# Improbable-AI/walk-these-ways

Hardware: AMD Instinct MI355X
Metric: env-steps/sec (sim+PPO) (higher is better)
Workload: dtype f32

## Files before the change

walk-these-ways_amd/csrc/go1ppo.hip:

```cpp
#include <hip/hip_runtime.h>
#include <stdint.h>
#include <string.h>
#include "../../include/go1ppo.h"

typedef uint16_t bf16_t;
static_assert(sizeof(Go1PpoAdamExtras) == 56 && sizeof(Go1PpoGemmArgs) == 96 && sizeof(Go1PpoWgradProblem) == 96 && sizeof(Go1PpoGradPiece) == 56, "ctypes mirrors (fused.py) assume these sizes");
typedef __attribute__((ext_vector_type(4))) float f32x4;

__device__ __forceinline__ float bf2f(bf16_t u) { return __uint_as_float(((uint32_t)u) << 16); }
__device__ __forceinline__ bf16_t f2bf(float f) {
  return __builtin_bit_cast(bf16_t, (__bf16)f);
}
struct alignas(16) Bf8 { bf16_t v[8]; };

typedef __attribute__((ext_vector_type(4))) uint32_t u32x4_t;
__device__ __forceinline__ void put16_wt(void* p, u32x4_t v) {
  asm volatile("global_store_dwordx4 %0, %1, off sc1\n\ts_nop 1" : : "v"((__attribute__((address_space(1))) void*)p), "v"(v) : "memory");
}
__device__ __forceinline__ void put16_wt(void* p, const Bf8& v) { put16_wt(p, __builtin_bit_cast(u32x4_t, v)); }
__device__ __forceinline__ void put16_wt(void* p, f32x4 v) { put16_wt(p, __builtin_bit_cast(u32x4_t, v)); }
__device__ __forceinline__ void put16_wt(void* p, uint4 v) { put16_wt(p, u32x4_t{v.x, v.y, v.z, v.w}); }

__device__ __forceinline__ float elu1(float x) {
  float em = x > -1e-3f ? fmaf(0.5f * x, x, x) : __expf(x) - 1.f;
// ... 501 lines not shown
  wgrad2_body((const bf16_t*)P.dz, P.ld_dz, (const bf16_t*)P.h, P.ld_h, m_begin, m_end, P.dW, P.ldw, P.bias_grad, n0, k0,
              P.bias_grad && k0 == 0, T, P.zero_n, P.zero_k0, P.zero_k1);
}

__global__ __launch_bounds__(256) void act_kernel(const bf16_t* mean, const bf16_t* value, int head_ld, const float* std, int A,
                                                  int64_t rows, const float* noise, float* actions, float* mu, float* sigma,
                                                  float* values, float* logp) {
  int64_t r = (int64_t)blockIdx.x * blockDim.x + threadIdx.x;
  if (r >= rows) return;
  const float HALF_LOG_2PI = 0.9189385332046727f;
  float lp = 0.f, logs = 0.f;
  for (int j = 0; j < A; j++) {
    float sg = std[j], m = bf2f(mean[r * head_ld + j]);
    float a = m + sg * noise[r * A + j];
    float z = (a - m) / sg;
    lp += -0.5f * z * z;
    logs += logf(sg);
    actions[r * A + j] = a;
    mu[r * A + j] = m;
    sigma[r * A + j] = sg;
  }
  logp[r] = lp - (logs + A * HALF_LOG_2PI);
  values[r] = bf2f(value[r * head_ld]);
}

__global__ __launch_bounds__(256) void store_step_kernel(const float* rewards, const uint8_t* dones, const uint8_t* time_outs,
                                                         const int32_t* env_bins, const float* values, float gamma, int64_t n,
                                                         float* rewards_out, uint8_t* dones_out, float* env_bins_out) {
  int64_t i = (int64_t)blockIdx.x * 256 + threadIdx.x;
  if (i >= n) return;
  float r = rewards[i];
  if (time_outs) r += gamma * (values[i] * (time_outs[i] ? 1.f : 0.f));
  rewards_out[i] = r;
  dones_out[i] = dones[i];
  if (env_bins) env_bins_out[i] = (float)env_bins[i];
}

__global__ __launch_bounds__(256) void gae_kernel(const float* rewards, const uint8_t* dones, const float* values, const float* last_values,
                                                  int T, int64_t N, float gamma, float lam, float* returns, float* advantages, double* stats) {
  __shared__ double red[2][4];
  int64_t e = (int64_t)blockIdx.x * 256 + threadIdx.x;
  double s1 = 0.0, s2 = 0.0;
  if (e < N) {
    float adv = 0.f, next_v = last_values[e];
    for (int t = T - 1; t >= 0; t--) {
      const int64_t i = (int64_t)t * N + e;
      const float alive = 1.f - (float)dones[i];
      const float v = values[i];
      const float delta = rewards[i] + alive * gamma * next_v - v;
      adv = delta + alive * gamma * lam * adv;
      const float ret = adv + v;
      const float a = ret - v;
      returns[i] = ret;
      advantages[i] = a;
      s1 += a;
      s2 += (double)a * a;
      next_v = v;
    }
  }
  for (int o = 32; o > 0; o >>= 1) { s1 += __shfl_xor(s1, o, 64); s2 += __shfl_xor(s2, o, 64); }
  if ((threadIdx.x & 63) == 0) { red[0][threadIdx.x >> 6] = s1; red[1][threadIdx.x >> 6] = s2; }
  __syncthreads();
  if (threadIdx.x < 2) det_put(det_gae_slab + (int64_t)blockIdx.x * 2 + threadIdx.x, red[threadIdx.x][0] + red[threadIdx.x][1] + red[threadIdx.x][2] + red[threadIdx.x][3]);
  if (!det_last(&det_count[DET_GAE], gridDim.x)) return;
  if (threadIdx.x < 2) {
    double t = 0.0;
#pragma unroll 16
    for (unsigned b = 0; b < gridDim.x; b++) t += det_gae_slab[(int64_t)b * 2 + threadIdx.x];
    stats[threadIdx.x] += t;
  }
}

__global__ __launch_bounds__(256) void normalize_kernel(float* adv, int64_t n, const double* stats) {
  int64_t i = (int64_t)blockIdx.x * 256 + threadIdx.x;
  if (i >= n) return;
  const double cnt = stats[2], mean = stats[0] / cnt;
  double var = (stats[1] - cnt * mean * mean) / (cnt - 1.0);
  var = var > 0.0 ? var : 0.0;
  const float m = (float)mean, sd = (float)sqrt(var);
  adv[i] = (adv[i] - m) / (sd + 1e-8f);
}

#define OPT_BLOCKS 2048
template <bool NORM>
__device__ __forceinline__ float grad_pieces_pass(float* g, int64_t n, const Go1PpoGradPiece* __restrict__ pieces, int num_pieces, float gscale) {
  const int64_t tid = (int64_t)blockIdx.x * 256 + threadIdx.x, nth = (int64_t)gridDim.x * 256;
  auto gap_groups = [&](int64_t lo, int64_t hi) -> int64_t { return NORM && hi > lo ? (hi - lo + 7) >> 3 : 0; };
  auto piece_groups = [&](const Go1PpoGradPiece& P) -> int64_t { return P.kind == 0 ? gap_groups(P.begin, P.begin + P.count) : P.count >> 3; };
  int64_t total = 0;
  {
    int64_t cur = 0;
    for (int q = 0; q <= num_pieces; q++) {
      const int64_t pb = q < num_pieces ? pieces[q].begin : n;
      total += gap_groups(cur, pb < n ? pb : n);
      if (q == num_pieces) break;
      total += piece_groups(pieces[q]);
      cur = pieces[q].begin + pieces[q].count;
    }
  }
  float s = 0.f;
  auto plain8 = [&](int64_t i, int64_t hi) {
    if (i + 8 <= hi) {
      const f32x4 a = reinterpret_cast<const f32x4*>(g + i)[0] * gscale, b = reinterpret_cast<const f32x4*>(g + i)[1] * gscale;
#pragma unroll
      for (int e = 0; e < 4; e++) { s = fmaf(a[e], a[e], s); s = fmaf(b[e], b[e], s); }
    } else {
      for (int64_t j = i; j < hi; j++) { const float x = g[j] * gscale; s = fmaf(x, x, s); }
    }
  };
  for (int64_t f = tid; f < total; f += nth) {
    int64_t cum = 0, cur = 0;
    for (int q = 0; q <= num_pieces; q++) {
      const int64_t pb = q < num_pieces ? pieces[q].begin : n, ge = pb < n ? pb : n;
      const int64_t gg = gap_groups(cur, ge);
      if (f >= cum && f < cum + gg) plain8(cur + ((f - cum) << 3), ge);
      cum += gg;
      if (q == num_pieces) break;
      const Go1PpoGradPiece P = pieces[q];
      const int64_t pg = piece_groups(P);
      cur = P.begin + P.count;
      if (f >= cum && f < cum + pg) {
        const int64_t i = (f - cum) << 3;
        if (P.kind == 0) plain8(P.begin + i, cur);
        else {
          float acc[8] = {0.f, 0.f, 0.f, 0.f, 0.f, 0.f, 0.f, 0.f};
          if (P.kind == 1) {
            const float* src = (const float*)P.src + i;
            int b = 0;
            for (; b + 4 <= P.slabs; b += 4) {
              f32x4 lo[4], hi[4];
#pragma unroll
              for (int u = 0; u < 4; u++) {
                lo[u] = reinterpret_cast<const f32x4*>(src + (int64_t)(b + u) * P.stride)[0];
                hi[u] = reinterpret_cast<const f32x4*>(src + (int64_t)(b + u) * P.stride)[1];
              }
#pragma unroll
              for (int u = 0; u < 4; u++)
#pragma unroll
                for (int e = 0; e < 4; e++) { acc[e] += lo[u][e]; acc[4 + e] += hi[u][e]; }
            }
            for (; b < P.slabs; b++) {
              const f32x4 lo = reinterpret_cast<const f32x4*>(src + (int64_t)b * P.stride)[0], hi = reinterpret_cast<const f32x4*>(src + (int64_t)b * P.stride)[1];
#pragma unroll
              for (int e = 0; e < 4; e++) { acc[e] += lo[e]; acc[4 + e] += hi[e]; }
            }
          } else {
            const bf16_t* src = (const bf16_t*)P.src + i;
            int b = 0;
            for (; b + 4 <= P.slabs; b += 4) {
              Bf8 v[4];
#pragma unroll
              for (int u = 0; u < 4; u++) v[u] = *reinterpret_cast<const Bf8*>(src + (int64_t)(b + u) * P.stride);
#pragma unroll
              for (int u = 0; u < 4; u++)
#pragma unroll
                for (int e = 0; e < 8; e++) acc[e] += bf2f(v[u].v[e]);
            }
            for (; b < P.slabs; b++) {
              const Bf8 v = *reinterpret_cast<const Bf8*>(src + (int64_t)b * P.stride);
#pragma unroll
              for (int e = 0; e < 8; e++) acc[e] += bf2f(v.v[e]);
            }
          }
          if (P.zero_rows > 0) {
            const int64_t row = i / P.cols;
            const int c = (int)(i - row * P.cols);
            if (row < P.zero_rows && c < P.zero_c1 && c + 8 > P.zero_c0) {
#pragma unroll
              for (int e = 0; e < 8; e++)
                if (c + e >= P.zero_c0 && c + e < P.zero_c1) acc[e] = 0.f;
            }
          }
          float* out = g + P.begin + i;
          reinterpret_cast<f32x4*>(out)[0] = f32x4{acc[0], acc[1], acc[2], acc[3]};
          reinterpret_cast<f32x4*>(out)[1] = f32x4{acc[4], acc[5], acc[6], acc[7]};
          if (NORM) {
#pragma unroll
            for (int e = 0; e < 8; e++) { const float x = acc[e] * gscale; s = fmaf(x, x, s); }
          }
        }
      }
      cum += pg;
    }
  }
  return s;
}
__global__ __launch_bounds__(256) void grad_reduce_kernel(float* g, const Go1PpoGradPiece* __restrict__ pieces, int num_pieces) {
  grad_pieces_pass<false>(g, 0, pieces, num_pieces, 1.f);
}

__global__ __launch_bounds__(256) void prestep_kernel(const float* g, int64_t n, float gscale, float* partial, float* step, float* lr,
                                                      const float* kl, float kl_scale, float desired_kl, float lr_min, float lr_max,
                                                      const Go1PpoGradPiece* __restrict__ pieces, int num_pieces) {
  __shared__ float red[4];
  float s = 0.f;
  if (partial && pieces) {
    s = grad_pieces_pass<true>(const_cast<float*>(g), n, pieces, num_pieces, gscale);
    for (int o = 32; o > 0; o >>= 1) s += __shfl_xor(s, o, 64);
    if ((threadIdx.x & 63) == 0) red[threadIdx.x >> 6] = s;
    __syncthreads();
    if (threadIdx.x == 0) partial[blockIdx.x] = red[0] + red[1] + red[2] + red[3];
  } else if (partial) {
    const int64_t n4 = ((reinterpret_cast<uintptr_t>(g) & 15) == 0) ? n >> 2 : 0;
    for (int64_t i = (int64_t)blockIdx.x * 256 + threadIdx.x; i < n4; i += (int64_t)OPT_BLOCKS * 256) {
      const f32x4 x = reinterpret_cast<const f32x4*>(g)[i] * gscale;
      s = fmaf(x[0], x[0], s); s = fmaf(x[1], x[1], s); s = fmaf(x[2], x[2], s); s = fmaf(x[3], x[3], s);
    }
    for (int64_t i = 4 * n4 + (int64_t)blockIdx.x * 256 + threadIdx.x; i < n; i += (int64_t)OPT_BLOCKS * 256) {
      float x = g[i] * gscale;
      s = fmaf(x, x, s);
    }
    for (int o = 32; o > 0; o >>= 1) s += __shfl_xor(s, o, 64);
    if ((threadIdx.x & 63) == 0) red[threadIdx.x >> 6] = s;
    __syncthreads();
    if (threadIdx.x == 0) partial[blockIdx.x] = red[0] + red[1] + red[2] + red[3];
  }
  if (blockIdx.x == 0 && threadIdx.x == 0) {
    step[0] += 1.f;
    if (kl) {
      const float k = kl[0] * kl_scale, l = lr[0];
      if (k > desired_kl * 2.f) lr[0] = fmaxf(lr_min, l / 1.5f);
      else if (k < desired_kl / 2.f && k > 0.f) lr[0] = fminf(lr_max, l * 1.5f);
    }
  }
}

template <int V>
__global__ __launch_bounds__(256) void adam_kernel(float* p, float* g, float* m, float* v, int64_t start0, int64_t count0,
                                                   int64_t start1, int64_t count1, float gscale, const float* partial, float max_norm,
                                                   const float* step, const float* lr, float beta1, float beta2, float eps,
                                                   bf16_t* body, int64_t n_body, float* tail, int64_t n_tail, int zero_grad, float* zero_slot,
                                                   Go1PpoAdamExtras ex) {
  __shared__ float clip_red[4];
  float clip = 1.f;
  if (partial) {
    float s = 0.f;
#pragma unroll
    for (int u = 0; u < OPT_BLOCKS / 256; u++) s += partial[threadIdx.x + 256 * u];
    for (int o = 32; o > 0; o >>= 1) s += __shfl_xor(s, o, 64);
    if ((threadIdx.x & 63) == 0) clip_red[threadIdx.x >> 6] = s;
    __syncthreads();
    clip = fminf(1.f, max_norm / (sqrtf((clip_red[0] + clip_red[1]) + (clip_red[2] + clip_red[3])) + 1e-6f));
  }
  const float gs = gscale * clip;
  const float t = step[0], l = lr[0];
  const float bc1 = 1.f - powf(beta1, t), bc2 = 1.f - powf(beta2, t);
  const float step_size = l / bc1, inv_sqrt_bc2 = rsqrtf(bc2);
  const int64_t total = count0 + count1;
// ... 559 lines not shown
```

walk-these-ways_amd/go1_gym_learn/ppo_cse/fused.py:

```python
import ctypes
import os

import torch

HEAD = 64
_HERE = os.path.dirname(os.path.abspath(__file__))
_LIB_PATH = os.path.normpath(os.path.join(_HERE, "..", "..", "csrc", "libgo1ppo.so"))
_lib = None


class Go1PpoLibraryMissing(RuntimeError):
    pass


class LossArgs(ctypes.Structure):
    _fields_ = [("mean", ctypes.c_void_p), ("value", ctypes.c_void_p), ("std", ctypes.c_void_p),
                ("head_ld", ctypes.c_int32), ("num_actions", ctypes.c_int32), ("rows", ctypes.c_int64),
                ("idx", ctypes.c_void_p), ("actions", ctypes.c_void_p), ("old_mu", ctypes.c_void_p),
                ("old_sigma", ctypes.c_void_p), ("old_logp", ctypes.c_void_p), ("advantages", ctypes.c_void_p),
                ("returns", ctypes.c_void_p), ("old_values", ctypes.c_void_p),
                ("clip_param", ctypes.c_float), ("value_loss_coef", ctypes.c_float), ("entropy_coef", ctypes.c_float),
                ("use_clipped_value_loss", ctypes.c_int32),
                ("d_mean", ctypes.c_void_p), ("d_value", ctypes.c_void_p), ("d_std", ctypes.c_void_p),
                ("d_mean_bias", ctypes.c_void_p), ("d_value_bias", ctypes.c_void_p), ("kl", ctypes.c_void_p),
# ... 111 lines not shown
    L.go1ppo_normalize.argtypes = [vp, i64, vp, vp]
    L.go1ppo_opt_partials.argtypes = []
    L.go1ppo_opt_prestep.argtypes = [vp, i64, f32, vp, vp, vp, vp, f32, f32, f32, f32, vp]
    L.go1ppo_opt_prestep_pieces.argtypes = [vp, i64, vp, i32, f32, vp, vp, vp, vp, f32, f32, f32, f32, vp]
    L.go1ppo_grad_reduce.argtypes = [vp, vp, i32, vp]
    L.go1ppo_opt_adam.argtypes = [vp, vp, vp, vp, i64, i64, i64, i64, f32, vp, f32, vp, vp, f32, f32, f32, vp, i64, vp, i64, i32, vp,
                                  ctypes.POINTER(AdamExtras), vp]
    for name in EXPORTED_SYMBOLS[:-1]:
        getattr(L, name).restype = ctypes.c_int
    L.go1ppo_version.restype = ctypes.c_char_p
    if path is None:
        _lib = L
    return L


def _stream():
    return torch.cuda.current_stream().cuda_stream


def _chk(rc, what):
    if rc != 0:
        raise RuntimeError(f"{what} failed with code {rc}")


def _ptr(t):
    return None if t is None else t.data_ptr()


def _ld(t):
    assert t.dim() == 2 and t.stride(1) == 1
    return t.stride(0)


def gemm_args(a, b, c, bias=None, elu=None, elu_bwd_of=None, elu_skip=None):
    g = GemmArgs()
    g.A, g.B, g.C, g.bias, g.H = a.data_ptr(), b.data_ptr(), c.data_ptr(), _ptr(bias), _ptr(elu_bwd_of)
    g.M, g.N, g.K, g.lda, g.ldb, g.ldc = a.shape[0], b.shape[0], a.shape[1], _ld(a), _ld(b), _ld(c)
    assert b.shape[1] == g.K and tuple(c.shape) == (g.M, g.N) and (elu is None or elu_bwd_of is None)
    assert a.dtype == b.dtype == c.dtype == torch.bfloat16 and (bias is None or bias.dtype in (torch.float32, torch.bfloat16))
    g.bias_bf16 = int(bias is not None and bias.dtype == torch.bfloat16)
    if elu_bwd_of is not None:
        assert elu_bwd_of.shape == c.shape and elu_bwd_of.dtype == torch.bfloat16
        g.epilogue, g.ldh = 2, _ld(elu_bwd_of)
    elif elu is not None:
        g.epilogue = 1
        g.elu_c0, g.elu_c1 = (0, g.N) if elu is True else elu
        if elu_skip is not None:
            g.elu_skip_c0, g.elu_skip_c1 = elu_skip
    return g


def gemm_nt(lib, a, b, c, bias=None, elu=None, elu_bwd_of=None):
    g = gemm_args(a, b, c, bias, elu, elu_bwd_of)
    _chk(lib.go1ppo_gemm_nt(ctypes.byref(g), _stream()), "go1ppo_gemm_nt")
    return c


def gemm_nt_pair(lib, first, second):
    ga, gb = gemm_args(**first), gemm_args(**second)
    _chk(lib.go1ppo_gemm_nt_pair(ctypes.byref(ga), ctypes.byref(gb), _stream()), "go1ppo_gemm_nt_pair")


class FusedNet:

    def __init__(self, policy, body, grad, M, lib, with_grad, two_streams=True, fused_tails=None):
        assert body.dtype == torch.bfloat16 and body.is_cuda
        self.pol, self.M, self.lib = policy, M, lib
        dev = body.device
        self.P = {name: policy._block(body, name) for name, _ in policy.blocks}
        self.G = {name: policy._block(grad, name) for name, _ in policy.blocks} if grad is not None else None
        self.nd, self.na, self.nc = policy.first
        self.n1 = self.nd + self.na + self.nc
        self.depth = {n: len(l) for n, l in policy.nets.items()}
        bf = dict(device=dev, dtype=torch.bfloat16)
        self.Y1 = torch.zeros(M, self.n1, **bf)
        self.Y1d = torch.zeros(M, self.nd, **bf)
        self.Z = {n: {li: torch.zeros(M, self.P[f"{n}.{li}.W"].shape[0], **bf) for li in range(1, d)}
                  for n, d in self.depth.items()}
        assert policy.npv <= HEAD and self.P["Wz"].shape == (self.na, HEAD)
        self._recording, self._batched, self._plans = None, False, {}
        self._grad = grad
        self.defer_grad_sum = False
        self._rec_pieces, self._slab_ws, self._last_pieces = None, {}, {}
        self._wgrad_tn = M % 64 == 0
        self._tails = self._tails_ad = None
        if fused_tails is None:
            fused_tails = M <= int(os.environ.get("GO1_FUSED_TAILS_MAX_ROWS", "2048"))
        self._elu_on_load = not with_grad
        if fused_tails and self._fused_tails_ok():
            nd, na = self.nd, self.na
            eol = self._elu_on_load
            self._tails = (self._tail_args([("adaptation", self.Y1[:, :nd])], with_grad, elu_in=eol),
                           self._tail_args([("actor", self.Y1[:, nd:nd + na]), ("critic", self.Y1[:, nd + na:])], with_grad, elu_in=eol,
                                           latent_for="actor" if eol else None))
            self._tails_ad = self._tail_args([("adaptation", self.Y1d)], with_grad)
        self._mlp2 = (self._tails is None and os.environ.get("GO1_MLP2", "1") == "1" and self.nd == MLP2_DIMS[0] and
                      all(self.depth[n] >= 3 and tuple(self.P[f"{n}.{self.depth[n] - 2}.W"].shape) == (MLP2_DIMS[1], MLP2_DIMS[0])
                          and tuple(self.P[f"{n}.{self.depth[n] - 1}.W"].shape) == (MLP2_DIMS[2], MLP2_DIMS[1]) for n in self.depth)
                      and self.depth["adaptation"] == 3 and self.depth["actor"] == 4 and self.depth["critic"] == 4)
        self._mlp2_cache = {}
        self._tail_in_loss = False
        na1, nc1 = int(self.P["actor.1.W"].shape[0]), int(self.P["critic.1.W"].shape[0])
        nt_ok = all(v % 64 == 0 for v in (na1, nc1, self.na, self.n1 - self.nd - self.na)) and \
            all(self.P[k].data_ptr() % 16 == 0 for k in ("actor.1.b", "critic.1.b", "actor.1.W", "critic.1.W"))
        pair_ok = nt_ok and na1 == nc1 and self.na == self.n1 - self.nd - self.na
        self._l1_nt = nt_ok
        self._pair = pair_ok
        self._side = torch.cuda.Stream(device=dev) if two_streams else None
        if with_grad:
            self.X = torch.zeros(M, policy.Kp, **bf)
            self.dH1 = {"adaptation": torch.zeros(M, self.nd, **bf), "actor": torch.zeros(M, self.na, **bf),
                        "critic": torch.zeros(M, self.nc, **bf)}
            self.dY1 = torch.zeros(M, self.n1, **bf)
            self.dZ = {n: {li: torch.zeros_like(z) for li, z in zs.items()} for n, zs in self.Z.items()}
            w1_split = next((b for b in (M // 6144, 4, 2) if b >= 2 and M % b == 0 and (M // b) % 64 == 0), 1)
            self._w1_tmp = torch.zeros(w1_split, self.n1, policy.Kp, **bf)
            self._dgrad_nt = self._mlp2 and nt_ok
            self._WT = {n: torch.zeros(self.P[f"{n}.1.W"].shape[1], self.P[f"{n}.1.W"].shape[0], **bf) for n in ("actor", "critic")} \
                if self._dgrad_nt else None
            self._wt_by_optimizer = False
            self.priv_mask = (self.nd + self.na, policy.K + 1, policy.K + 1 + policy.npv)

    def _elu(self, y, lat=None, lat_cols=0):
        wz = self.P["Wz"] if lat is not None else None
        _chk(self.lib.go1ppo_elu_fwd(y.data_ptr(), y.shape[0], y.shape[1], _ld(y), _ptr(lat), _ld(lat) if lat is not None else 0,
                                     self.pol.npv if lat is not None else 0, _ptr(wz), HEAD, lat_cols, _stream()), "go1ppo_elu_fwd")

    def _elu_bwd(self, d, h, bias_grad, out=None):
        out = d if out is None else out
        _chk(self.lib.go1ppo_elu_bwd(d.data_ptr(), _ld(d), _ptr(h), _ld(h) if h is not None else 0, d.shape[0], d.shape[1],
                                     _ptr(bias_grad), out.data_ptr(), _ld(out), _stream()), "go1ppo_elu_bwd")

    def _wgrad(self, dz, h, gW, gb=None, zero=None):
        n, k = dz.shape[1], h.shape[1]
        assert gW.shape == (n, k) and gW.is_contiguous()
        if self._recording is not None:
            self._recording.append((dz, h, gW, gb, zero))
            return
        if self._batched:
            return
        assert zero is None or zero[0] == 0, "the structural zeros are applied by the batched launch"
        _chk(self.lib.go1ppo_wgrad(dz.data_ptr(), _ld(dz), h.data_ptr(), _ld(h), dz.shape[0], n, k, gW.data_ptr(), k, _ptr(gb),
                                   _stream()), "go1ppo_wgrad")

    def _tail_args(self, nets_and_inputs, keep_intermediates, elu_in=False, latent_for=None):
        a = TailArgs()
        a.num_nets = len(nets_and_inputs)
        for N, (net, h) in zip(a.net, nets_and_inputs):
            d = self.depth[net]
            N.in_, N.rows, N.ld_in, N.num_layers = h.data_ptr(), h.shape[0], _ld(h), d - 1
            N.elu_in = int(bool(elu_in))
            if elu_in and latent_for == net:
                lat, wz = self.Z["adaptation"][self.depth["adaptation"] - 1], self.P["Wz"]
                N.latent, N.wz, N.lat_ld, N.wz_ld, N.npv = lat.data_ptr(), wz.data_ptr(), _ld(lat), HEAD, self.pol.npv
            for li in range(1, d):
                L, W, z = N.layer[li - 1], self.P[f"{net}.{li}.W"], self.Z[net][li]
                last = li == d - 1
                L.W, L.bias = W.data_ptr(), self.P[f"{net}.{li}.b"].data_ptr()
                L.out = z.data_ptr() if (last or keep_intermediates) else None
                L.n_out, L.k_in, L.ld_out, L.elu = W.shape[0], W.shape[1], _ld(z), 0 if last else 1
        return a

    def _fused_tails_ok(self):
        ok = all(self.depth[n] - 1 <= 4 for n in self.depth)
        for n, d in self.depth.items():
            for li in range(1, d):
# ... 164 lines not shown
        nd, d, G, Z, dZ = self.nd, self.dH1["adaptation"], self.G, self.Z, self.dZ
        if not self._tail_in_loss:
            self._mlp2_bwd("adaptation_only", [("adaptation", self.Y1d, d)])
        self._wgrad(dZ["adaptation"][2], Z["adaptation"][1], G["adaptation.2.W"], None)
        self._wgrad(dZ["adaptation"][1], self.Y1d, G["adaptation.1.W"], G["adaptation.1.b"])
        self._big_wgrad(d, x, G["W1"][:nd], self._w1_tmp[:, :nd], own_kernel=self._wgrad_tn)

    def adam_transposes(self):
        if not getattr(self, "_dgrad_nt", False):
            return []
        out = []
        for n in ("actor", "critic"):
            i = self.pol.index[f"{n}.1.W"]
            rows, cols = self.pol.blocks[i][1]
            out.append((self.pol.offsets[i], rows, cols, self._WT[n]))
        return out

    def refresh_transposes(self):
        if getattr(self, "_dgrad_nt", False):
            for n in ("actor", "critic"):
                self._WT[n].copy_(self.P[f"{n}.1.W"].t())

    def _branch(self):
        if self._side is None:
            import contextlib
            return contextlib.nullcontext()
        self._side.wait_stream(torch.cuda.current_stream())
        self._forked = True
        return torch.cuda.stream(self._side)

    def _join(self):
        if self._side is not None and getattr(self, "_forked", False):
            torch.cuda.current_stream().wait_stream(self._side)
            self._forked = False

    def forward_adaptation(self, x):
        if self._mlp2:
            return self._forward_adaptation_mlp2(x)
        torch.mm(x, self.P["W1"][:self.nd].t(), out=self.Y1d)
        self._elu(self.Y1d)
        if self._tails_ad is not None:
            _chk(self.lib.go1ppo_tail_fwd(ctypes.byref(self._tails_ad), _stream()), "go1ppo_tail_fwd")
            return self.Z["adaptation"][self.depth["adaptation"] - 1]
        return self._tail("adaptation", self.Y1d)

    def _tail_bwd(self, net, h0, dh0, head_bias_done=True):
        P, G, d = self.P, self.G, self.depth[net]
        for li in range(d - 1, 0, -1):
            dz = self.dZ[net][li]
            h_in = self.Z[net][li - 1] if li > 1 else h0
            gb = None if (li == d - 1 and head_bias_done) else G[f"{net}.{li}.b"]
            self._wgrad(dz, h_in, G[f"{net}.{li}.W"], gb)
            out = self.dZ[net][li - 1] if li > 1 else dh0
            torch.mm(dz, P[f"{net}.{li}.W"], out=out)
            if li > 1:
                self._elu_bwd(out, h_in, None)

    def _big_wgrad(self, dY, x, gW, tmp, own_kernel=False):
        zr, zc0, zc1 = self.priv_mask
        zr = min(zr, gW.shape[0])
        if own_kernel:
            self._wgrad(dY, x, gW, zero=(zr, zc0, zc1))
            return
        b = tmp.shape[0]
        if b == 1 or not tmp.is_contiguous():
            torch.mm(dY.t(), x, out=tmp[0])
            part, count, stride = tmp[0], 1, gW.numel()
        else:
            torch.bmm(dY.view(b, dY.shape[0] // b, dY.shape[1]).transpose(1, 2), x.view(b, x.shape[0] // b, x.shape[1]), out=tmp)
            part, count, stride = tmp, b, tmp.stride(0)
        assert gW.is_contiguous() and part.stride(-1) == 1 and part.stride(-2) == gW.shape[1]
        if self._rec_pieces is not None:
            self._rec_pieces.append(dict(begin=self._grad_offset(gW), count=gW.numel(), src=part, stride=stride, kind=2, slabs=count,
                                         cols=gW.shape[1], zero=(zr, zc0, zc1)))

    def _grad_offset(self, view):
        off = (view.data_ptr() - self._grad.data_ptr()) // 4
        assert view.dtype == torch.float32 and view.is_contiguous() and 0 <= off and off + view.numel() <= self._grad.numel()
        return int(off)

    def last_pieces(self, kind):
        return self._last_pieces.get(kind)

    def _run_planned(self, key, fn):
        if key not in self._plans:
            self._recording, self._rec_pieces = [], []
            fn()
            rec, self._recording = self._recording, None
            pieces, self._rec_pieces = self._rec_pieces, None
            tab = (WgradProblem * len(rec))()
            for P, (dz, h, gW, gb, zero) in zip(tab, rec):
                P.dz, P.h, P.dW, P.bias_grad = dz.data_ptr(), h.data_ptr(), gW.data_ptr(), _ptr(gb)
                if zero is not None:
                    P.zero_n, P.zero_k0, P.zero_k1 = zero
                P.rows, P.ld_dz, P.ld_h, P.n, P.k, P.ldw = dz.shape[0], _ld(dz), _ld(h), dz.shape[1], h.shape[1], gW.shape[1]
            tn = self._wgrad_tn and all(P.rows % 64 == 0 and P.n % 8 == 0 and P.k % 8 == 0 for P in tab)
            plan = self.lib.go1ppo_wgrad_tn_plan if tn else self.lib.go1ppo_wgrad_plan
            if tn:
                for P, (dz, h, gW, gb, zero) in zip(tab, rec):
                    P.partials, P.partial_stride = 16, gW.numel()
            total = plan(tab, len(rec))
            if total <= 0:
                raise RuntimeError(f"go1ppo_wgrad_plan failed with code {total}")
            if tn:
                for j, (P, (dz, h, gW, gb, zero)) in enumerate(zip(tab, rec)):
                    S = -(-P.rows // P.chunk_rows)
                    ws = self._slab_ws.get((key[0], j))
                    if ws is None or tuple(ws.shape) != (S, gW.numel()):
                        ws = self._slab_ws[(key[0], j)] = torch.zeros(S, gW.numel(), device=gW.device, dtype=torch.float32)
                    P.partials, P.partial_stride = ws.data_ptr(), gW.numel()
                    pieces.append(dict(begin=self._grad_offset(gW), count=gW.numel(), src=ws, stride=gW.numel(), kind=1, slabs=S, cols=gW.shape[1],
                                       zero=(0, 0, 0)))
                if plan(tab, len(rec)) != total:
                    raise RuntimeError("go1ppo_wgrad_tn_plan: the plan changed with the slab buffers attached")
            dev = torch.frombuffer(bytearray(bytes(tab)), dtype=torch.uint8).to(self.Y1.device)
            ptab = None
            if pieces:
                pieces.sort(key=lambda q: q["begin"])
                arr = (GradPiece * len(pieces))()
                end = 0
                for A, q in zip(arr, pieces):
                    assert q["begin"] >= end and q["begin"] % 8 == 0 and q["count"] % 8 == 0 and q["stride"] % 8 == 0, "slab pieces: ascending, disjoint, multiples of 8"
                    end = q["begin"] + q["count"]
                    A.begin, A.count, A.src, A.stride, A.kind, A.slabs, A.cols = q["begin"], q["count"], q["src"].data_ptr(), q["stride"], q["kind"], q["slabs"], q["cols"]
                    A.zero_rows, A.zero_c0, A.zero_c1 = q["zero"]
                ptab = (torch.frombuffer(bytearray(bytes(arr)), dtype=torch.uint8).to(self.Y1.device), len(pieces), [q["src"] for q in pieces])
            self._plans[key] = (dev, len(rec), total, rec, tn, ptab)
        else:
            self._batched = True
            try:
                fn()
            finally:
                self._batched = False
        dev, count, total, _, tn, ptab = self._plans[key]
        launch = self.lib.go1ppo_wgrad_tn_batched if tn else self.lib.go1ppo_wgrad_batched
        _chk(launch(dev.data_ptr(), count, total, _stream()), "go1ppo_wgrad_batched")
        self._last_pieces[key[0]] = None
        if ptab is None:
            return
        if self.defer_grad_sum:
            self._last_pieces[key[0]] = ptab[:2]
        else:
            _chk(self.lib.go1ppo_grad_reduce(self._grad.data_ptr(), ptab[0].data_ptr(), ptab[1], _stream()), "go1ppo_grad_reduce")

    def backward(self, x):
        self._run_planned(("ppo", x.data_ptr()), lambda: (self._backward_mlp2 if self._mlp2 else self._backward)(x))

    def backward_adaptation(self, x):
        self._run_planned(("adaptation", x.data_ptr()), lambda: (self._backward_adaptation_mlp2 if self._mlp2 else self._backward_adaptation)(x))

    def _backward(self, x):
        nd, na = self.nd, self.na
        G, Y1, dY1, dH1 = self.G, self.Y1, self.dY1, self.dH1
        cols = {"adaptation": slice(0, nd), "actor": slice(nd, nd + na), "critic": slice(nd + na, self.n1)}
        with self._branch():
            self._tail_bwd("critic", Y1[:, cols["critic"]], dH1["critic"])
            self._elu_bwd(dH1["critic"], Y1[:, cols["critic"]], None, out=dY1[:, cols["critic"]])
        self._tail_bwd("actor", Y1[:, cols["actor"]], dH1["actor"])
        self._elu_bwd(dH1["actor"], Y1[:, cols["actor"]], None, out=dY1[:, cols["actor"]])
        last = self.depth["adaptation"] - 1
        latent, dlat = self.Z["adaptation"][last], self.dZ["adaptation"][last]
        dA1 = dY1[:, cols["actor"]]
        self._wgrad(dA1, latent, G["Wz"])
        torch.mm(dA1, self.P["Wz"], out=dlat)
        self._tail_bwd("adaptation", Y1[:, :nd], dH1["adaptation"], head_bias_done=False)
        self._elu_bwd(dH1["adaptation"], Y1[:, :nd], None, out=dY1[:, :nd])
        self._join()
        self._big_wgrad(dY1, x, G["W1"], self._w1_tmp)

    def _backward_adaptation(self, x):
        nd, d = self.nd, self.dH1["adaptation"]
        self._tail_bwd("adaptation", self.Y1d, d)
        self._elu_bwd(d, self.Y1d, None)
        self._big_wgrad(d, x, self.G["W1"][:nd], self._w1_tmp[:, :nd], own_kernel=self._wgrad_tn)

    def ppo_loss(self, st, idx, std, g_std, A, kl, acc):
        la, lc = self.depth["actor"] - 1, self.depth["critic"] - 1
        flat = lambda t: t.flatten(0, 1)
        a = LossArgs()
        a.mean, a.value, a.std = self.Z["actor"][la].data_ptr(), self.Z["critic"][lc].data_ptr(), std.data_ptr()
        a.head_ld, a.num_actions, a.rows = HEAD, std.numel(), self.M
        a.idx = idx.data_ptr()
        for field, t in (("actions", st.actions), ("old_mu", st.mu), ("old_sigma", st.sigma), ("old_logp", st.actions_log_prob),
                         ("advantages", st.advantages), ("returns", st.returns), ("old_values", st.values)):
            t = flat(t)
            assert t.is_contiguous() and t.dtype == torch.float32
            setattr(a, field, t.data_ptr())
        a.clip_param, a.value_loss_coef, a.entropy_coef = A.clip_param, A.value_loss_coef, A.entropy_coef
        a.use_clipped_value_loss = int(A.use_clipped_value_loss)
        a.d_mean, a.d_value = self.dZ["actor"][la].data_ptr(), self.dZ["critic"][lc].data_ptr()
        a.d_std = g_std.data_ptr()
        a.d_mean_bias = self.G[f"actor.{la}.b"].data_ptr()
        a.d_value_bias = self.G[f"critic.{lc}.b"].data_ptr()
        a.kl = kl.data_ptr()
        a.value_loss = acc[0:].data_ptr()
        a.surrogate_loss = acc[1:].data_ptr()
        if self._tail_in_loss:
            Z, dZ = self.Z, self.dZ
            arr = self._mlp2_tail("ac", [("actor", Z["actor"][1], dZ["actor"][1]), ("critic", Z["critic"][1], dZ["critic"][1])])
            _chk(self.lib.go1ppo_mlp2_tail_ppo(arr, ctypes.byref(a), _stream()), "go1ppo_mlp2_tail_ppo")
            return
        _chk(self.lib.go1ppo_loss(ctypes.byref(a), _stream()), "go1ppo_loss")

    def adaptation_loss(self, st, idx, num_train, selective, acc):
        last = self.depth["adaptation"] - 1
        pred, dpred = self.Z["adaptation"][last], self.dZ["adaptation"][last]
        target = st.privileged_observations.flatten(0, 1)
        assert target.is_contiguous() and target.dtype == torch.float32 and target.shape[1] == self.pol.npv
        if self._tail_in_loss:
            arr = self._mlp2_tail("adaptation_only", [("adaptation", self.Y1d, self.dH1["adaptation"])])
            q = MseArgs()
            q.target, q.idx, q.num_train, q.npv, q.selective = target.data_ptr(), idx.data_ptr(), num_train, self.pol.npv, int(selective)
            q.d_pred_bias, q.train_loss, q.test_loss = self.G[f"adaptation.{last}.b"].data_ptr(), acc[2:].data_ptr(), acc[3:].data_ptr()
            _chk(self.lib.go1ppo_mlp2_tail_mse(arr, ctypes.byref(q), _stream()), "go1ppo_mlp2_tail_mse")
            return
        _chk(self.lib.go1ppo_mse(pred.data_ptr(), HEAD, target.data_ptr(), self.pol.npv, idx.data_ptr(), self.M, num_train,
                                 int(selective), dpred.data_ptr(), self.G[f"adaptation.{last}.b"].data_ptr(),
                                 acc[2:].data_ptr(), acc[3:].data_ptr(), _stream()), "go1ppo_mse")


def act(lib, mean, value, std, noise, st, s):
    _chk(lib.go1ppo_act(mean.data_ptr(), value.data_ptr(), _ld(mean), std.data_ptr(), std.numel(), mean.shape[0], noise.data_ptr(),
                        st.actions[s].data_ptr(), st.mu[s].data_ptr(), st.sigma[s].data_ptr(), st.values[s].data_ptr(),
                        st.actions_log_prob[s].data_ptr(), _stream()), "go1ppo_act")


def store_step(lib, st, s, rewards, dones, time_outs, env_bins, gamma):
    n = rewards.shape[0]
    for t, dt in ((rewards, torch.float32), (dones, torch.uint8)):
        assert t.is_contiguous() and t.dtype == dt and t.shape[0] == n
    if time_outs is not None:
        assert time_outs.is_contiguous() and time_outs.element_size() == 1
    if env_bins is not None:
        assert env_bins.is_contiguous() and env_bins.dtype == torch.int32
    _chk(lib.go1ppo_store_step(rewards.data_ptr(), dones.data_ptr(), _ptr(time_outs), _ptr(env_bins), st.values[s].data_ptr(), gamma, n,
                               st.rewards[s].data_ptr(), st.dones[s].data_ptr(), st.env_bins[s].data_ptr() if env_bins is not None else None,
                               _stream()), "go1ppo_store_step")


def ring_step(lib, st, s, obs, privileged_obs, obs_history, X):
    N, no, H = st.num_envs, st.obs_ring.shape[2], st.history_length
    npv = st.privileged_observations.shape[-1]
    for t in (obs, privileged_obs):
        assert t.dtype == torch.float32 and t.is_contiguous() and t.shape[0] == N
    assert X.dtype == torch.bfloat16 and X.is_contiguous() and tuple(X.shape) == (N, st.padded_width)
    if s == 0:
        assert obs_history.dtype == torch.float32 and obs_history.stride(1) == 1 and tuple(obs_history.shape) == (N, H * no)
        _chk(lib.go1ppo_ring_snapshot(obs_history.data_ptr(), obs_history.stride(0), N, H, no, st.obs_ring.data_ptr(), _stream()),
             "go1ppo_ring_snapshot")
    dst = None if s == 0 else st.obs_ring[s + H - 1].data_ptr()
    _chk(lib.go1ppo_ring_step(obs.data_ptr(), privileged_obs.data_ptr(), dst, st.obs_ring[s].data_ptr(), N, H, no, npv, st.padded_width,
                              X.data_ptr(), st.observations[s].data_ptr(), st.privileged_observations[s].data_ptr(), _stream()),
         "go1ppo_ring_step")


def ring_gather(lib, st, idx, X):
    N, no, H = st.num_envs, st.obs_ring.shape[2], st.history_length
    priv = st.privileged_observations
    assert idx.dtype == torch.int64 and idx.is_contiguous() and X.is_contiguous() and tuple(X.shape) == (idx.numel(), st.padded_width)
    assert priv.dtype == torch.float32 and priv.is_contiguous()
    _chk(lib.go1ppo_ring_gather(st.obs_ring.data_ptr(), priv.data_ptr(), idx.data_ptr(), idx.numel(), N, H, no, priv.shape[-1],
                                st.padded_width, X.data_ptr(), _stream()), "go1ppo_ring_gather")


def gae(lib, st, last_values, gamma, lam, stats):
    T, N = st.num_transitions_per_env, st.num_envs
    stats.zero_()
    _chk(lib.go1ppo_gae(st.rewards.data_ptr(), st.dones.data_ptr(), st.values.data_ptr(), last_values.data_ptr(), T, N, gamma, lam,
                        st.returns.data_ptr(), st.advantages.data_ptr(), stats.data_ptr(), _stream()), "go1ppo_gae")
    stats[2] = float(T * N)


def normalize(lib, st, stats):
    _chk(lib.go1ppo_normalize(st.advantages.data_ptr(), st.advantages.numel(), stats.data_ptr(), _stream()), "go1ppo_normalize")


class FusedAdam:

    def __init__(self, lib, master, body, std, n_body, lr, ranges=None, betas=(0.9, 0.999), eps=1e-8):
        self.lib, self.master, self.body, self.std, self.n_body = lib, master, body, std, n_body
        dev = master.device
        self.m, self.v = torch.zeros_like(master), torch.zeros_like(master)
        self.step = torch.zeros(1, device=dev)
        self.lr = torch.full((1,), float(lr), device=dev)
        self.partial = torch.zeros(lib.go1ppo_opt_partials(), device=dev)
        self.betas, self.eps = betas, eps
        r = list(ranges or [(0, master.numel())]) + [(0, 0)]
        self.r0, self.r1 = r[0], r[1]
        self.n_norm = max(a + b for a, b in r)
        self.extras = AdamExtras()
        self._keep = []
# ... 35 lines not shown
```

Baseline: 5.308 million.

## Use wave-level prefix table for grad pieces and trim adaptation wgrad rows

The gradient-piece pass now builds a per-wave prefix-sum table of segment group counts using shuffles and ballots. Each wave then visits only the segments its 64 lanes cover, instead of every thread walking all pieces linearly. The zero-row division uses 32-bit math when sizes allow. Separately, the adaptation backward's weight-gradient plan limits rows to the training subset, rounded up to 64, so held-out rows are skipped; this adds plan-cache keys per row count and assumes held-out rows contribute zero gradient.

```diff
diff --git a/walk-these-ways_amd/csrc/go1ppo.hip b/walk-these-ways_amd/csrc/go1ppo.hip
--- a/walk-these-ways_amd/csrc/go1ppo.hip
+++ b/walk-these-ways_amd/csrc/go1ppo.hip
@@ -607,22 +607,44 @@
 }
 
 #define OPT_BLOCKS 2048
+__device__ __forceinline__ int64_t wave_uniform(int64_t x) {
+  return (int64_t)(((uint64_t)(uint32_t)__builtin_amdgcn_readfirstlane((int)((uint64_t)x >> 32)) << 32) |
+                   (uint32_t)__builtin_amdgcn_readfirstlane((int)(uint32_t)x));
+}
 template <bool NORM>
 __device__ __forceinline__ float grad_pieces_pass(float* g, int64_t n, const Go1PpoGradPiece* __restrict__ pieces, int num_pieces, float gscale) {
-  const int64_t tid = (int64_t)blockIdx.x * 256 + threadIdx.x, nth = (int64_t)gridDim.x * 256;
+  const int lane = threadIdx.x & 63;
+  const int64_t wave0 = (int64_t)blockIdx.x * 256 + 64 * __builtin_amdgcn_readfirstlane((int)(threadIdx.x >> 6)), nth = (int64_t)gridDim.x * 256;
   auto gap_groups = [&](int64_t lo, int64_t hi) -> int64_t { return NORM && hi > lo ? (hi - lo + 7) >> 3 : 0; };
   auto piece_groups = [&](const Go1PpoGradPiece& P) -> int64_t { return P.kind == 0 ? gap_groups(P.begin, P.begin + P.count) : P.count >> 3; };
-  int64_t total = 0;
-  {
-    int64_t cur = 0;
+  auto gap_lo = [&](int q) -> int64_t { return q ? pieces[q - 1].begin + pieces[q - 1].count : 0; };
+  auto gap_hi = [&](int q) -> int64_t { const int64_t pb = q < num_pieces ? pieces[q].begin : n; return pb < n ? pb : n; };
+  const bool table = num_pieces < 64;
+  int64_t total = 0, gstart = 0, pstart = 0;
+  if (table) {
+    int64_t gg = 0, pg = 0;
+    if (lane <= num_pieces) {
+      gg = gap_groups(gap_lo(lane), gap_hi(lane));
+      if (lane < num_pieces) pg = piece_groups(pieces[lane]);
+    }
+    int64_t incl = gg + pg;
+#pragma unroll
+    for (int o = 1; o < 64; o <<= 1) {
+      const int64_t up = __shfl_up(incl, o, 64);
+      if (lane >= o) incl += up;
+    }
+    gstart = incl - (gg + pg);
+    pstart = gstart + gg;
+    total = wave_uniform(__shfl(incl, 63, 64));
+  } else {
     for (int q = 0; q <= num_pieces; q++) {
-      const int64_t pb = q < num_pieces ? pieces[q].begin : n;
-      total += gap_groups(cur, pb < n ? pb : n);
-      if (q == num_pieces) break;
-      total += piece_groups(pieces[q]);
-      cur = pieces[q].begin + pieces[q].count;
-    }
-  }
+      total += gap_groups(gap_lo(q), gap_hi(q));
+      if (q < num_pieces) total += piece_groups(pieces[q]);
+    }
+  }
+  auto segment_of = [&](int64_t f) -> int {
+    return __popcll(__ballot(gstart <= f)) + __popcll(__ballot(pstart <= f)) - 1;
+  };
   float s = 0.f;
   auto plain8 = [&](int64_t i, int64_t hi) {
     if (i + 8 <= hi) {
@@ -633,17 +655,26 @@
       for (int64_t j = i; j < hi; j++) { const float x = g[j] * gscale; s = fmaf(x, x, s); }
     }
   };
-  for (int64_t f = tid; f < total; f += nth) {
-    int64_t cum = 0, cur = 0;
-    for (int q = 0; q <= num_pieces; q++) {
-      const int64_t pb = q < num_pieces ? pieces[q].begin : n, ge = pb < n ? pb : n;
-      const int64_t gg = gap_groups(cur, ge);
-      if (f >= cum && f < cum + gg) plain8(cur + ((f - cum) << 3), ge);
-      cum += gg;
-      if (q == num_pieces) break;
+  for (int64_t f0 = wave0; f0 < total; f0 += nth) {
+    const int64_t f = f0 + lane;
+    int k0 = 0, k1 = 2 * num_pieces;
+    int64_t cum = 0;
+    if (table) {
+      k0 = segment_of(f0);
+      k1 = segment_of(f0 + 63 < total ? f0 + 63 : total - 1);
+      cum = wave_uniform(__shfl((k0 & 1) ? pstart : gstart, k0 >> 1, 64));
+    }
+    for (int k = k0; k <= k1; k++) {
+      const int q = k >> 1;
+      if (!(k & 1)) {
+        const int64_t lo = gap_lo(q), ge = gap_hi(q), gg = gap_groups(lo, ge);
+        if (f >= cum && f < cum + gg) plain8(lo + ((f - cum) << 3), ge);
+        cum += gg;
+        continue;
+      }
       const Go1PpoGradPiece P = pieces[q];
       const int64_t pg = piece_groups(P);
-      cur = P.begin + P.count;
+      const int64_t cur = P.begin + P.count;
       if (f >= cum && f < cum + pg) {
         const int64_t i = (f - cum) << 3;
         if (P.kind == 0) plain8(P.begin + i, cur);
@@ -688,7 +719,7 @@
             }
           }
           if (P.zero_rows > 0) {
-            const int64_t row = i / P.cols;
+            const int64_t row = (uint64_t)P.count >> 31 ? i / P.cols : (int64_t)((uint32_t)i / (uint32_t)P.cols);
             const int c = (int)(i - row * P.cols);
             if (row < P.zero_rows && c < P.zero_c1 && c + 8 > P.zero_c0) {
 #pragma unroll
diff --git a/walk-these-ways_amd/go1_gym_learn/ppo_cse/fused.py b/walk-these-ways_amd/go1_gym_learn/ppo_cse/fused.py
--- a/walk-these-ways_amd/go1_gym_learn/ppo_cse/fused.py
+++ b/walk-these-ways_amd/go1_gym_learn/ppo_cse/fused.py
@@ -217,6 +217,7 @@
         self._grad = grad
         self.defer_grad_sum = False
         self._rec_pieces, self._slab_ws, self._last_pieces = None, {}, {}
+        self._heldout_from = None
         self._wgrad_tn = M % 64 == 0
         self._tails = self._tails_ad = None
         if fused_tails is None:
@@ -547,7 +548,7 @@
     def last_pieces(self, kind):
         return self._last_pieces.get(kind)
 
-    def _run_planned(self, key, fn):
+    def _run_planned(self, key, fn, rows=None):
         if key not in self._plans:
             self._recording, self._rec_pieces = [], []
             fn()
@@ -559,6 +560,8 @@
                 if zero is not None:
                     P.zero_n, P.zero_k0, P.zero_k1 = zero
                 P.rows, P.ld_dz, P.ld_h, P.n, P.k, P.ldw = dz.shape[0], _ld(dz), _ld(h), dz.shape[1], h.shape[1], gW.shape[1]
+                if rows is not None:
+                    P.rows = min(P.rows, rows)
             tn = self._wgrad_tn and all(P.rows % 64 == 0 and P.n % 8 == 0 and P.k % 8 == 0 for P in tab)
             plan = self.lib.go1ppo_wgrad_tn_plan if tn else self.lib.go1ppo_wgrad_plan
             if tn:
@@ -612,7 +615,12 @@
         self._run_planned(("ppo", x.data_ptr()), lambda: (self._backward_mlp2 if self._mlp2 else self._backward)(x))
 
     def backward_adaptation(self, x):
-        self._run_planned(("adaptation", x.data_ptr()), lambda: (self._backward_adaptation_mlp2 if self._mlp2 else self._backward_adaptation)(x))
+        num_train, self._heldout_from = self._heldout_from, None
+        rows = None
+        if num_train is not None and num_train > 0 and self._wgrad_tn:
+            rows = min(self.M, -(-int(num_train) // 64) * 64)
+        self._run_planned(("adaptation", x.data_ptr()) + ((rows,) if rows is not None else ()),
+                          lambda: (self._backward_adaptation_mlp2 if self._mlp2 else self._backward_adaptation)(x), rows=rows)
 
     def _backward(self, x):
         nd, na = self.nd, self.na
@@ -672,6 +680,7 @@
         pred, dpred = self.Z["adaptation"][last], self.dZ["adaptation"][last]
         target = st.privileged_observations.flatten(0, 1)
         assert target.is_contiguous() and target.dtype == torch.float32 and target.shape[1] == self.pol.npv
+        self._heldout_from = int(num_train)
         if self._tail_in_loss:
             arr = self._mlp2_tail("adaptation_only", [("adaptation", self.Y1d, self.dH1["adaptation"])])
             q = MseArgs()
```

Result: no change. 5.281 million (-0.5%).
